# noamteyssier/sgcount

Hardware: NVIDIA B200
Metric: reads/sec matched per B200 (kernel & end-to-end) (higher is better)
Workload: dtype u8

## Files before the change

### sgcount_b200/csrc/common.cuh

```cuda
#pragma once

#include <cuda_runtime.h>
#include <stdint.h>

namespace sgc {

constexpr uint32_t kMaxK = 30;
constexpr uint32_t kNarrowMaxK = 20;
constexpr int kSeeds = 3;
constexpr int32_t kMiss = -1;

constexpr uint64_t kDirKindInline = 1ull << 62, kDirKindRun = 2ull << 62;
constexpr int kDirKindShift = 62;
constexpr uint32_t kDirStartMask = 0x3FFFFFu;

constexpr int kPostIdxShift = 40;

constexpr uint64_t kFrontFlag = 1ull << 40;
constexpr uint64_t kFrontOccupied = 1ull << 41;
constexpr int kFrontIdxShift = 42;

struct Key {
  uint32_t lo, hi;
};

__host__ __device__ __forceinline__ Key base_field(uint32_t j, bool wide) {
  const uint32_t word = j >> 2, byte = j & 3u;
  if (word < 4) return Key{3u << (8 * byte + 2 * word), 0u};
  return wide ? Key{0u, 3u << (8 * byte + 2 * (word - 4))} : Key{0u, 3u << (2 * byte)};
}
__host__ __device__ __forceinline__ void key_set_base(Key& k, uint32_t j, bool wide, uint32_t code) {
  const Key f = base_field(j, wide);
  k.lo = (k.lo & ~f.lo) | ((f.lo & (~f.lo + 1)) * code);
  k.hi = (k.hi & ~f.hi) | ((f.hi & (~f.hi + 1)) * code);
}
__host__ __device__ __forceinline__ uint32_t key_get_base(Key k, uint32_t j, bool wide) {
  const Key f = base_field(j, wide);
  return f.lo ? (k.lo & f.lo) / (f.lo & (~f.lo + 1)) : (k.hi & f.hi) / (f.hi & (~f.hi + 1));
}

constexpr uint32_t kFixedPartsMinK = 17;
struct SeedParts {
  uint32_t end[2];
  uint32_t keep_lo[kSeeds], keep_hi[kSeeds];
};
inline SeedParts make_seed_parts(uint32_t k, bool wide) {
  SeedParts sp{};
  const bool fixed = k >= kFixedPartsMinK;
  const uint32_t p0 = fixed ? 8 : (k + 2) / 3, p1 = fixed ? 8 : (k - p0 + 1) / 2;
  sp.end[0] = p0;
  sp.end[1] = p0 + p1;
  for (uint32_t j = 0; j < k; ++j) {
    const int part = j < sp.end[0] ? 0 : (j < sp.end[1] ? 1 : 2);
    const Key f = base_field(j, wide);
    for (int i = 0; i < kSeeds; ++i)
      if (i != part) {
        sp.keep_lo[i] |= f.lo;
        sp.keep_hi[i] |= f.hi;
      }
  }
  return sp;
}
__host__ __device__ __forceinline__ Key seed_of(const SeedParts& sp, Key k, int i) {
  return Key{k.lo & sp.keep_lo[i], k.hi & sp.keep_hi[i]};
}
__host__ __device__ __forceinline__ int part_of_base(const SeedParts& sp, uint32_t j) {
  return j < sp.end[0] ? 0 : (j < sp.end[1] ? 1 : 2);
}

template <bool FIXED>
__host__ __device__ __forceinline__ Key seed_of_t(const SeedParts& sp, Key k, int i) {
  if (FIXED) return i == 0 ? Key{k.lo & 0xF0F0F0F0u, k.hi} : (i == 1 ? Key{k.lo & 0x0F0F0F0Fu, k.hi} : Key{k.lo, 0u});
  return seed_of(sp, k, i);
}
template <bool FIXED>
__host__ __device__ __forceinline__ int part_of_base_t(const SeedParts& sp, uint32_t j) {
  if (FIXED) return j < 8 ? 0 : (j < 16 ? 1 : 2);
  return part_of_base(sp, j);
}
template <bool FIXED>
__host__ __device__ __forceinline__ uint32_t kept_difference(const SeedParts& sp, Key x, int list) {
  if (FIXED) {
    const uint32_t keep_lo = list == 0 ? 0xF0F0F0F0u : (list == 1 ? 0x0F0F0F0Fu : 0xFFFFFFFFu);
    return (x.lo & keep_lo) | (list < 2 ? x.hi : 0u);
  }
  return (x.lo & sp.keep_lo[list]) | (x.hi & sp.keep_hi[list]);
}

__host__ __device__ __forceinline__ uint32_t seed_hash(Key s) {
  uint32_t h = s.lo * 0x9E3779B1u + s.hi * 0x85EBCA77u;
  h ^= h >> 15;
  return h * 0x2C1B3C6Du;
}
__host__ __device__ __forceinline__ uint32_t front_hash(uint32_t lo, uint32_t hi) {
  return lo * 0x9E3779B1u + hi * 0x85EBCA77u;
}

__host__ __device__ __forceinline__ bool is_acgt(uint8_t c) {
  return c == 'A' || c == 'C' || c == 'G' || c == 'T';
}
__host__ __device__ __forceinline__ uint32_t code_of(uint8_t c) { return (c >> 1) & 3u; }

struct IndexView {
  const uint64_t* __restrict__ dir64[kSeeds];
  const ulonglong2* __restrict__ dir128[kSeeds];
  const uint64_t* __restrict__ post;
  const uint64_t* __restrict__ front;
};

struct LibView {
  uint32_t k, n;
  uint32_t wide;
  uint32_t dir_shift;
  uint32_t front_shift;
  SeedParts parts;
  IndexView fwd;
  IndexView rev;
};

#ifdef __CUDACC__

#ifndef SGC_L1_HINT
#define SGC_L1_HINT ""
#endif
__device__ __forceinline__ uint64_t ldg_u64(const uint64_t* p, uint64_t policy) {
  uint64_t v;
  asm volatile("ld.global.nc" SGC_L1_HINT ".L2::cache_hint.u64 %0, [%1], %2;" : "=l"(v) : "l"(p), "l"(policy));
  return v;
}
__device__ __forceinline__ uint32_t ldg_u32(const uint32_t* p, uint64_t policy) {
  uint32_t v;
  asm volatile("ld.global.nc" SGC_L1_HINT ".L2::cache_hint.u32 %0, [%1], %2;" : "=r"(v) : "l"(p), "l"(policy));
  return v;
}
__device__ __forceinline__ ulonglong2 ldg_u128(const ulonglong2* p, uint64_t policy) {
  ulonglong2 v;
  asm volatile("ld.global.nc" SGC_L1_HINT ".L2::cache_hint.v2.u64 {%0,%1}, [%2], %3;"
               : "=l"(v.x), "=l"(v.y)
               : "l"(p), "l"(policy));
  return v;
}
__device__ __forceinline__ void load_bucket(const uint64_t* p, uint64_t (&w)[4], uint64_t policy) {
  asm volatile("ld.global.nc" SGC_L1_HINT ".L2::cache_hint.v4.u64 {%0,%1,%2,%3}, [%4], %5;"
               : "=l"(w[0]), "=l"(w[1]), "=l"(w[2]), "=l"(w[3])
               : "l"(p), "l"(policy));
}
__device__ __forceinline__ uint64_t l2_evict_first_policy() {
  uint64_t pol;
  asm volatile("createpolicy.fractional.L2::evict_first.b64 %0, 1.0;" : "=l"(pol));
  return pol;
}
__device__ __forceinline__ uint64_t l2_evict_last_policy() {
  uint64_t pol;
  asm volatile("createpolicy.fractional.L2::evict_last.b64 %0, 1.0;" : "=l"(pol));
  return pol;
}

__device__ __forceinline__ int bases_differing(Key x) {
  return __popc((x.lo | (x.lo >> 1)) & 0x55555555u) + __popc((x.hi | (x.hi >> 1)) & 0x55555555u);
}

struct SeedRun {
  uint32_t first;
  uint32_t count;
};
__device__ __forceinline__ SeedRun seed_run128(const LibView& v, int seed, ulonglong2 entry) {
  SeedRun r;
  r.first = (uint32_t)seed * v.n + ((uint32_t)entry.y & kDirStartMask);
  r.count = (entry.x >> kDirKindShift) == 2 ? (uint32_t)(entry.y >> 22) : 0u;
  return r;
}
__device__ __forceinline__ SeedRun seed_run64(const LibView& v, int seed, uint64_t entry) {
  SeedRun r;
  r.first = (uint32_t)seed * v.n + ((uint32_t)entry & kDirStartMask);
  r.count = (entry >> kDirKindShift) == 2 ? (uint32_t)(entry >> 22) : 0u;
  return r;
}
template <bool WIDE>
__device__ __forceinline__ void load_posting(const IndexView& ix, uint32_t at, uint64_t policy, Key& key, uint32_t& idx) {
  if (WIDE) {
    const uint64_t w = ldg_u64(ix.post + 2 * (size_t)at, policy);
    key = Key{(uint32_t)w, (uint32_t)(w >> 32)};
    idx = (uint32_t)ldg_u64(ix.post + 2 * (size_t)at + 1, policy);
  } else {
    const uint64_t w = ldg_u64(ix.post + at, policy);
    key = Key{(uint32_t)w, (uint32_t)(w >> 32) & 0xFFu};
    idx = (uint32_t)(w >> kPostIdxShift) & 0x3FFFFFu;
  }
}

template <bool WIDE, typename F>
__device__ __forceinline__ void for_each_posting(const LibView& v, const IndexView& ix, int seed, Key key,
                                                 uint64_t policy, F&& visit) {
  const uint32_t h = seed_hash(seed_of(v.parts, key, seed));
  SeedRun r;
  if (WIDE) {
    const ulonglong2 e = ldg_u128(ix.dir128[seed] + (h >> v.dir_shift), policy);
    if ((e.x >> kDirKindShift) == 1) {
      visit(Key{(uint32_t)e.x, (uint32_t)(e.x >> 32) & 0x3FFFFFFFu}, (uint32_t)e.y);
      return;
    }
    r = seed_run128(v, seed, e);
  } else {
    const uint64_t e = ldg_u64(ix.dir64[seed] + (h >> v.dir_shift), policy);
    if ((e >> kDirKindShift) == 1) {
      visit(Key{(uint32_t)e, (uint32_t)(e >> 32) & 0xFFu}, (uint32_t)(e >> kPostIdxShift) & 0x3FFFFFu);
      return;
    }
    r = seed_run64(v, seed, e);
  }
#pragma unroll 1
  for (uint32_t c = 0; c < r.count; ++c) {
    Key mk;
    uint32_t idx;
    load_posting<WIDE>(ix, r.first + c, policy, mk, idx);
    if (visit(mk, idx)) break;
  }
}

template <bool WIDE, bool FIXED = false>
__device__ __forceinline__ int32_t lookup_token(const LibView& v, const IndexView& ix, bool with_perm, Key key, Key hole,
                                                int hole_list, bool active, int* kind, uint64_t policy) {
  static_assert(kSeeds == 3, "written for three lists");
  const bool wild = hole_list >= 0;
  int32_t found = kMiss;
  int parents = 0;
  bool member = false;
  auto consider = [&](int list, Key mk, uint32_t idx) {
    const Key x{(mk.lo ^ key.lo) & ~hole.lo, (mk.hi ^ key.hi) & ~hole.hi};
    if (kept_difference<FIXED>(v.parts, x, list) != 0) return;
    if ((x.lo | x.hi) == 0) {
      if (wild) {
        ++parents;
      } else {
        member = true;
      }
      found = (int32_t)idx;
    } else if (!wild && !member && bases_differing(x) == 1) {
      ++parents;
      found = (int32_t)idx;
    }
  };
  bool use[kSeeds];
  uint32_t h[kSeeds];
  SeedRun r[kSeeds];
#pragma unroll
  for (int i = 0; i < kSeeds; ++i) {
    use[i] = active && (wild ? i == hole_list : (i == 0 || with_perm));
    h[i] = seed_hash(seed_of_t<FIXED>(v.parts, key, i));
  }
  if (WIDE) {
    ulonglong2 entry[kSeeds];
#pragma unroll
    for (int i = 0; i < kSeeds; ++i)
      entry[i] = use[i] ? ldg_u128(ix.dir128[i] + (h[i] >> v.dir_shift), policy) : ulonglong2{0ull, 0ull};
#pragma unroll
    for (int i = 0; i < kSeeds; ++i) {
      if ((entry[i].x >> kDirKindShift) == 1)
        consider(i, Key{(uint32_t)entry[i].x, (uint32_t)(entry[i].x >> 32) & 0x3FFFFFFFu}, (uint32_t)entry[i].y);
      r[i] = seed_run128(v, i, entry[i]);
    }
  } else {
    uint64_t entry[kSeeds];
#pragma unroll
    for (int i = 0; i < kSeeds; ++i) entry[i] = use[i] ? ldg_u64(ix.dir64[i] + (h[i] >> v.dir_shift), policy) : 0ull;
#pragma unroll
    for (int i = 0; i < kSeeds; ++i) {
      if ((entry[i] >> kDirKindShift) == 1)
        consider(i, Key{(uint32_t)entry[i], (uint32_t)(entry[i] >> 32) & 0xFFu},
                 (uint32_t)(entry[i] >> kPostIdxShift) & 0x3FFFFFu);
      r[i] = seed_run64(v, i, entry[i]);
    }
  }
  const uint32_t end0 = r[0].count, end1 = end0 + r[1].count, total = end1 + r[2].count;
  const uint32_t base0 = r[0].first, base1 = r[1].first - end0, base2 = r[2].first - end1;
#pragma unroll 1
  for (uint32_t j = 0; j < total && !member; ++j) {
    const bool in0 = j < end0, in1 = j < end1;
    const uint32_t at = (in0 ? base0 : (in1 ? base1 : base2)) + j;
    Key mk;
    uint32_t idx;
    load_posting<WIDE>(ix, at, policy, mk, idx);
    consider(in0 ? 0 : (in1 ? 1 : 2), mk, idx);
  }
  if (member) {
    if (kind) *kind = 1;
    return found;
  }
  if (with_perm && parents == 1) {
    if (kind) *kind = 2;
    return found;
  }
  return kMiss;
}

template <bool WIDE>
__device__ __forceinline__ int32_t lookup_clean(const LibView& v, const IndexView& ix, bool with_perm, Key key,
                                                int* kind, uint64_t policy) {
  return lookup_token<WIDE>(v, ix, with_perm, key, Key{0u, 0u}, -1, true, kind, policy);
}

template <bool WIDE>
__device__ __forceinline__ int32_t lookup_wild(const LibView& v, const IndexView& ix, Key key, uint32_t pos, int* kind,
                                               uint64_t policy) {
  const Key hole = base_field(pos, WIDE);
  key.lo &= ~hole.lo;
  key.hi &= ~hole.hi;
  return lookup_token<WIDE>(v, ix, true, key, hole, part_of_base(v.parts, pos), true, kind, policy);
}

template <bool WIDE>
__device__ __forceinline__ int32_t window_lookup_t(const LibView& v, const IndexView& ix, bool with_perm, Key key,
                                                   int nbad, uint32_t bad_pos, bool bad_is_wild, int* kind,
                                                   uint64_t policy) {
  if (nbad == 0) return lookup_clean<WIDE>(v, ix, with_perm, key, kind, policy);
  if (nbad == 1 && bad_is_wild && with_perm) return lookup_wild<WIDE>(v, ix, key, bad_pos, kind, policy);
  return kMiss;
}

#endif

}
```

### sgcount_b200/csrc/count.cu

```cuda
#include <algorithm>
#include <cstdlib>
#include <mutex>
#include <set>
#include <utility>
#include <vector>

#include "internal.h"

namespace sgc {
namespace {

struct StreamGeom {
  int k, n, o;
  uint32_t with_perm;
  int win_src;
  int lead;
  uint32_t shift_bits[3];
  uint32_t try_plus, try_minus;
  int n_words;
  uint32_t last_mask;
  uint32_t wild_byte;
};

inline StreamGeom make_geom(uint32_t k, uint32_t read_len, int offset, bool with_perm, bool reverse, bool recursion,
                            int rc_mode) {
  StreamGeom g;
  g.k = (int)k;
  g.n = (int)read_len;
  g.o = offset;
  g.with_perm = with_perm;
  g.try_plus = recursion && g.o + 1 + g.k <= g.n;
  g.try_minus = g.try_plus && g.o >= 1;
  g.win_src = reverse ? g.n - g.o - g.k : g.o;
  const int d_plus = reverse ? -1 : 1;
  const bool before = (g.try_plus && d_plus < 0) || (g.try_minus && d_plus > 0);
  g.lead = before ? 1 : 0;
  g.shift_bits[0] = 8u * (uint32_t)g.lead;
  g.shift_bits[1] = 8u * (uint32_t)(g.lead + d_plus);
  g.shift_bits[2] = 8u * (uint32_t)(g.lead - d_plus);
  g.n_words = (g.k + 3) >> 2;
  g.last_mask = (g.k & 3) ? ((1u << (8 * (g.k & 3))) - 1) : ~0u;
  g.wild_byte = (reverse && rc_mode == SGC_RC_BITTRICK) ? (uint32_t)'J' : (uint32_t)'N';
  return g;
}

constexpr int kHotGuides = 4;

struct CountParams {
  LibView lib;
  const uint8_t* lines;
  const uint8_t* lines_end;
  const uint32_t* line_off;
  const uint32_t* line_end;
  uint64_t n_reads;
  uint64_t first_read;
  uint32_t stride, read_len;
  int offset;
  uint8_t with_perm, reverse, recursion, rc_mode;
  unsigned long long* state;
  unsigned long long* rep;
  uint32_t n_rep;
  uint32_t n_guides;
  int32_t hot[kHotGuides];
  uint32_t off_base;
  int32_t* assign_out;
  uint32_t debug;
  uint32_t zero;
  StreamGeom geom;
};

struct HotCounts {
  uint32_t c[kHotGuides];
};

template <int MODE>
__device__ __forceinline__ void flush_matched(const CountParams& p, uint32_t matched, const HotCounts& hot) {
  matched = __reduce_add_sync(0xffffffffu, matched);
  if ((threadIdx.x & 31) == 0 && matched) atomicAdd(p.state + p.n_guides + 1, (unsigned long long)matched);
  if (MODE == 4) {
#pragma unroll
    for (int j = 0; j < kHotGuides; ++j) {
      const uint32_t h = __reduce_add_sync(0xffffffffu, hot.c[j]);
      if ((threadIdx.x & 31) == 0 && h) atomicAdd(p.state + p.hot[j], (unsigned long long)h);
    }
  }
  if (blockIdx.x == 0 && threadIdx.x == 0) atomicAdd(p.state + p.n_guides, (unsigned long long)p.n_reads);
}

template <int MODE>
__device__ __forceinline__ void count_hit(const CountParams& p, unsigned long long* my_counts, int32_t hit,
                                          uint32_t& matched, HotCounts& hot) {
  if (hit >= 0) {
    ++matched;
    if (MODE == 4) {
      bool is_hot = false;
#pragma unroll
      for (int j = 0; j < kHotGuides; ++j) {
        const bool h = hit == p.hot[j];
        hot.c[j] += h;
        is_hot |= h;
      }
      if (!is_hot) atomicAdd(my_counts + hit, 1ull);
    } else {
      if (MODE != 2 || !(p.debug & 1u)) atomicAdd((MODE == 3 ? my_counts : p.state) + hit, 1ull);
    }
  }
}

__global__ void fold_replicas_kernel(unsigned long long* __restrict__ state, unsigned long long* __restrict__ rep,
                                     uint32_t n, uint32_t n_rep) {
  const uint32_t i = blockIdx.x * blockDim.x + threadIdx.x;
  if (i >= n) return;
  unsigned long long sum = 0;
  for (uint32_t r = 0; r < n_rep; ++r) {
    const unsigned long long v = rep[(size_t)r * n + i];
    if (v) {
      sum += v;
      rep[(size_t)r * n + i] = 0;
    }
  }
  if (sum) state[i] += sum;
}

constexpr int kWarpReads = 32;
constexpr int kMaxStages = 4;
#ifndef SGC_HANDBACK_MBAR
#define SGC_HANDBACK_MBAR 0
#endif
constexpr int kQueueCap = 64;
constexpr uint32_t kReadIdxBits = 30;

__device__ __forceinline__ uint32_t smem_u32(const void* p) { return (uint32_t)__cvta_generic_to_shared(p); }

__device__ __forceinline__ void mbar_init(uint64_t* bar, uint32_t count) {
  asm volatile("mbarrier.init.shared::cta.b64 [%0], %1;" ::"r"(smem_u32(bar)), "r"(count));
}
__device__ __forceinline__ void mbar_expect_tx(uint32_t bar, uint32_t bytes) {
  asm volatile("mbarrier.arrive.expect_tx.shared::cta.b64 _, [%0], %1;" ::"r"(bar), "r"(bytes) : "memory");
}
__device__ __forceinline__ void mbar_arrive(uint32_t bar) {
  asm volatile("mbarrier.arrive.shared::cta.b64 _, [%0];" ::"r"(bar) : "memory");
}
__device__ __forceinline__ void mbar_wait(uint32_t bar, uint32_t parity) {
  asm volatile(
      "{\n"
      ".reg .pred p;\n"
      "WAIT_LOOP:\n"
      "mbarrier.try_wait.parity.shared::cta.b64 p, [%0], %1;\n"
      "@p bra WAIT_DONE;\n"
      "bra WAIT_LOOP;\n"
      "WAIT_DONE:\n"
      "}\n" ::"r"(bar),
      "r"(parity)
      : "memory");
}
__device__ __forceinline__ void bulk_load(uint32_t dst, const void* src, uint32_t bytes, uint32_t bar, uint64_t policy) {
  asm volatile(
      "cp.async.bulk.shared::cluster.global.mbarrier::complete_tx::bytes.L2::cache_hint [%0], [%1], %2, [%3], %4;" ::
          "r"(dst),
      "l"(src), "r"(bytes), "r"(bar), "l"(policy)
      : "memory");
}
__device__ __forceinline__ bool elect_one() {
  uint32_t pred;
  asm volatile("{\n.reg .pred p;\nelect.sync _|p, 0xffffffff;\nselp.u32 %0, 1, 0, p;\n}\n" : "=r"(pred));
  return pred != 0;
}
template <int OFFSET>
__device__ __forceinline__ uint32_t lds_u32(uint32_t addr) {
  uint32_t v;
  asm volatile("ld.shared.u32 %0, [%1+%2];" : "=r"(v) : "r"(addr), "n"(OFFSET) : "memory");
  return v;
}
template <int I, int N>
struct LoadWords {
  static __device__ __forceinline__ void run(uint32_t addr, uint32_t* W) {
    W[I] = lds_u32<4 * I>(addr);
    LoadWords<I + 1, N>::run(addr, W);
  }
};
template <int N>
struct LoadWords<N, N> {
  static __device__ __forceinline__ void run(uint32_t, uint32_t*) {}
};

__device__ __forceinline__ uint32_t nonzero_byte_flags(uint32_t x) {
  return (((x & 0x7F7F7F7Fu) + 0x7F7F7F7Fu) | x) & 0x80808080u;
}

__device__ __forceinline__ uint32_t ascii_residue(uint32_t w) {
  const uint32_t is_t = (w >> 2) & ~(w >> 1) & 0x01010101u;
  return ((w & 0xF9F9F9F9u) ^ (is_t * 0x11u)) ^ 0x41414141u;
}

template <int NW, bool WIDE>
__device__ __forceinline__ uint32_t pack_window(const uint32_t (&w)[NW], int n_words, uint32_t last_mask, Key& key,
                                                uint32_t (&x)[NW]) {
  uint32_t lo = 0, hi = 0, any = 0;
#pragma unroll
  for (int i = 0; i < NW; ++i) {
    x[i] = ascii_residue(w[i]);
    uint32_t c = (w[i] >> 1) & 0x03030303u;
    if (NW >= 5) {
      if (i == NW - 1) {
        x[i] &= last_mask;
        c &= last_mask;
      }
    } else {
      const uint32_t mk = i < n_words - 1 ? ~0u : (i == n_words - 1 ? last_mask : 0u);
      x[i] &= mk;
      c &= mk;
    }
    any |= x[i];
    if (i < 4)
      lo += c << (2 * i);
    else
      hi += c << (2 * (i - 4));
  }
  if (!WIDE) hi = (hi * 0x01041040u) >> 24;
  key = Key{lo, hi};
  return any;
}

template <int NW>
struct WarpQueueT {
  uint32_t w[NW + 1][kQueueCap];
  uint32_t tag[kQueueCap];
};

template <int NW, bool WIDE>
__device__ __forceinline__ int32_t try_position(const LibView& v, const IndexView& ix, const StreamGeom& g,
                                                const uint32_t (&S)[NW + 1], uint32_t shift, uint64_t policy,
                                                uint32_t debug = 0) {
  uint32_t w[NW], x[NW];
#pragma unroll
  for (int i = 0; i < NW; ++i) w[i] = __funnelshift_r(S[i], S[i + 1], shift);
  Key key;
  const uint32_t any = pack_window<NW, WIDE>(w, g.n_words, g.last_mask, key, x);
  if (debug & 8u) return (key.lo == 0x12345678u && any == 77u) ? 0 : kMiss;
  int nbad = 0;
  uint32_t bad_word = 0, bad_flags = 0, bad_w = 0;
#pragma unroll
  for (int i = 0; i < NW; ++i) {
    const uint32_t f = nonzero_byte_flags(x[i]);
    nbad += __popc(f);
    if (f) {
      bad_word = (uint32_t)i;
      bad_flags = f;
      bad_w = w[i];
    }
  }
  const uint32_t byte = ((uint32_t)(__ffs((int)bad_flags) - 8) >> 3) & 3u;
  const bool wild = g.with_perm && nbad == 1 && ((bad_w >> (8 * byte)) & 0xFFu) == g.wild_byte;
  const uint32_t pos = wild ? 4 * bad_word + byte : 0u;
  Key hole{0u, 0u};
  if (wild) {
    hole = base_field(pos, WIDE);
    key.lo &= ~hole.lo;
    key.hi &= ~hole.hi;
  }
  constexpr bool kFixedParts = NW == 5 || WIDE;
  static_assert(kFixedPartsMinK <= 17, "k = 17..30 must use the fixed parts");
  return lookup_token<WIDE, kFixedParts>(v, ix, g.with_perm, key, hole,
                                         wild ? part_of_base_t<kFixedParts>(v.parts, pos) : -1, any == 0 || wild,
                                         nullptr, policy);
}

__device__ __forceinline__ uint64_t ldg_stream_u64(const uint64_t* p, uint64_t policy) {
  uint64_t v;
  asm volatile("ld.global.nc.L2::cache_hint.u64 %0, [%1], %2;" : "=l"(v) : "l"(p), "l"(policy));
  return v;
}

constexpr uint32_t kLineIdxBits = 27;
constexpr uint32_t kLineLead = 1u << 27, kLinePlus = 1u << 28, kLineMinus = 1u << 29;
constexpr int kLineWarps = 8;

template <int NW, bool WIDE>
__global__ void __launch_bounds__(kLineWarps * 32) count_lines_kernel(CountParams p) {
  __shared__ WarpQueueT<NW> queues[kLineWarps];
  const int lane = threadIdx.x & 31, warp = threadIdx.x >> 5;
  WarpQueueT<NW>* q = &queues[warp];
  uint32_t matched = 0;
  HotCounts hot{};
  const uint64_t table_policy = l2_evict_last_policy();
  const uint64_t line_policy = l2_evict_first_policy();
  const int k = (int)p.lib.k;
  const StreamGeom& g = p.geom;
  const IndexView& ix = p.reverse ? p.lib.rev : p.lib.fwd;
  const uint32_t gwarp = blockIdx.x * kLineWarps + warp, gwarps = gridDim.x * kLineWarps;
  unsigned long long* my_counts = p.rep + (size_t)(gwarp & (p.n_rep - 1)) * p.n_guides;
  const int d_plus = p.reverse ? -1 : 1;
  constexpr int NL = (4 * NW + 11 + 7) / 8;
  static_assert(2 * NL >= NW + 3, "span words");
  uint32_t qn = 0;

  auto settle = [&](int32_t hit, uint32_t ridx) {
    if (p.assign_out) p.assign_out[p.first_read + ridx] = hit;
    count_hit<4>(p, my_counts, hit, matched, hot);
  };
  auto drain = [&](bool all) {
    while (qn >= 32 || (all && qn > 0)) {
      const uint32_t cnt = qn < 32 ? qn : 32;
      qn -= cnt;
      int next = -1;
      uint32_t S[NW + 1], tag = 0;
      if ((uint32_t)lane < cnt) {
        const uint32_t e = qn + lane;
#pragma unroll
        for (int i = 0; i < NW + 1; ++i) S[i] = q->w[i][e];
        tag = q->tag[e];
        const uint32_t pos = tag >> 30, ridx = tag & ((1u << kLineIdxBits) - 1);
        const int lead = (tag & kLineLead) ? 1 : 0;
        const uint32_t shift = 8u * (uint32_t)(pos == 0 ? lead : (pos == 1 ? lead + d_plus : lead - d_plus));
        const int32_t hit = try_position<NW, WIDE>(p.lib, ix, g, S, shift, table_policy);
        if (hit == kMiss) next = pos == 0 ? ((tag & kLinePlus) ? 1 : -1) : (pos == 1 && (tag & kLineMinus) ? 2 : -1);
        if (next < 0) settle(hit, ridx);
      }
      __syncwarp();
      const uint32_t pm = __ballot_sync(0xffffffffu, next >= 0);
      if (pm) {
        if (next >= 0) {
          const uint32_t e = qn + __popc(pm & ((1u << lane) - 1));
#pragma unroll
          for (int i = 0; i < NW + 1; ++i) q->w[i][e] = S[i];
          q->tag[e] = ((uint32_t)next << 30) | (tag & 0x3FFFFFFFu);
        }
        qn += __popc(pm);
      }
      __syncwarp();
    }
  };

  const uint64_t n_tiles = (p.n_reads + 31) / 32;
  for (uint64_t t = gwarp; t < n_tiles; t += gwarps) {
    const uint64_t i = t * 32 + lane;
    int park = -1;
    uint32_t S[NW + 1] = {}, flags = 0;
    if (i < p.n_reads) {
      const uint64_t r = p.first_read + i;
      uint64_t start;
      int n;
      if (p.line_end) {
        start = p.line_off[r];
        n = (int)(p.line_end[r] - p.line_off[r]);
      } else if (p.line_off) {
        const uint32_t a = p.line_off[r], b = p.line_off[r + 1];
        start = a - p.off_base;
        n = (int)(b - a) - 1;
      } else {
        start = r * p.stride;
        n = (int)p.read_len;
      }
      if (p.offset + k > n) {
        settle(kMiss, (uint32_t)i);
      } else {
        const bool try_plus = p.recursion && p.offset + 1 + k <= n;
        const bool try_minus = try_plus && p.offset >= 1;
        const int win_src = p.reverse ? n - p.offset - k : p.offset;
        const int lead = ((try_plus && d_plus < 0) || (try_minus && d_plus > 0)) ? 1 : 0;
        flags = (lead ? kLineLead : 0u) | (try_plus ? kLinePlus : 0u) | (try_minus ? kLineMinus : 0u);
        const uint8_t* sb = p.lines + start + win_src - lead;
        const uint64_t* a8 = reinterpret_cast<const uint64_t*>((uintptr_t)sb & ~(uintptr_t)7);
        uint32_t R[2 * NL];
#pragma unroll
        for (int j = 0; j < NL; ++j) {
          const uint64_t v =
              reinterpret_cast<const uint8_t*>(a8 + j) < p.lines_end ? ldg_stream_u64(a8 + j, line_policy) : 0ull;
          R[2 * j] = (uint32_t)v;
          R[2 * j + 1] = (uint32_t)(v >> 32);
        }
        const uint32_t sh = (uint32_t)((uintptr_t)sb & 7u);
        const bool odd = (sh & 4u) != 0;
        const uint32_t bits = (sh & 3u) * 8u;
#pragma unroll
        for (int j = 0; j < NW + 1; ++j) {
          const uint32_t w0 = odd ? R[j + 1] : R[j], w1 = odd ? R[j + 2] : R[j + 1];
          S[j] = __funnelshift_r(w0, w1, bits);
        }
        uint32_t w[NW], x[NW];
#pragma unroll
        for (int j = 0; j < NW; ++j) w[j] = __funnelshift_r(S[j], S[j + 1], 8u * (uint32_t)lead);
        Key key;
        const uint32_t any = pack_window<NW, WIDE>(w, g.n_words, g.last_mask, key, x);
        park = 0;
        if (any == 0) {
          uint64_t b[4];
          load_bucket(ix.front + (size_t)(front_hash(key.lo, key.hi) >> p.lib.front_shift) * 4, b, table_policy);
          bool found, flagged;
          int32_t idx;
          if (!WIDE) {
            uint32_t sel = 0;
#pragma unroll
            for (int j = 3; j >= 0; --j)
              if ((uint32_t)b[j] == key.lo) sel = (uint32_t)(b[j] >> 32);
            const uint32_t want = key.hi | (uint32_t)(kFrontOccupied >> 32);
            found = ((sel ^ want) & (0xFFu | (uint32_t)(kFrontOccupied >> 32))) == 0;
            idx = (int32_t)(sel >> (kFrontIdxShift - 32));
            flagged = (b[0] & kFrontFlag) != 0;
          } else {
            const uint64_t probe = ((uint64_t)key.hi << 32) | key.lo;
            const bool m0 = b[0] == probe && (b[1] & kFrontOccupied), m1 = b[2] == probe && (b[3] & kFrontOccupied);
            found = m0 || m1;
            idx = (int32_t)((m0 ? b[1] : b[3]) >> kFrontIdxShift);
            flagged = (b[1] & kFrontFlag) != 0;
          }
          if (found) {
            park = -1;
            settle(idx, (uint32_t)i);
          } else if (!flagged && !g.with_perm) {
            park = try_plus ? 1 : -1;
            if (park < 0) settle(kMiss, (uint32_t)i);
          }
        } else if (!g.with_perm) {
          park = try_plus ? 1 : -1;
          if (park < 0) settle(kMiss, (uint32_t)i);
        }
      }
    }
    const uint32_t pm = __ballot_sync(0xffffffffu, park >= 0);
    if (pm) {
      if (park >= 0) {
        const uint32_t e = qn + __popc(pm & ((1u << lane) - 1));
#pragma unroll
        for (int j = 0; j < NW + 1; ++j) q->w[j][e] = S[j];
        q->tag[e] = ((uint32_t)park << 30) | flags | (uint32_t)i;
      }
      qn += __popc(pm);
      __syncwarp();
    }
    drain(false);
  }
  drain(true);
  flush_matched<4>(p, matched, hot);
}

template <int NW, bool WIDE, int MODE>
__global__ void __launch_bounds__(384, 2) count_stream_kernel(const CountParams p, uint32_t n_wtiles, int n_stages,
                                                              uint32_t stage_bytes) {
  extern __shared__ __align__(128) uint8_t smem[];
  const int lane = threadIdx.x & 31;
  const int warp = __shfl_sync(0xffffffffu, (int)(threadIdx.x >> 5), 0);
  const int warps_per_cta = blockDim.x >> 5;
  uint8_t* my_tiles = smem + (size_t)warp * n_stages * stage_bytes;
  uint64_t* bars = reinterpret_cast<uint64_t*>(smem + (size_t)warps_per_cta * n_stages * stage_bytes);
  uint64_t* my_bar = bars + warp * (2 * kMaxStages);
  WarpQueueT<NW>* q = reinterpret_cast<WarpQueueT<NW>*>(bars + warps_per_cta * (2 * kMaxStages)) + warp;

  const uint32_t tile_bytes = kWarpReads * p.stride;
  const uint32_t gwarp = blockIdx.x * warps_per_cta + warp;
  const uint32_t gwarps = gridDim.x * warps_per_cta;
  const uint64_t src_step = (uint64_t)gwarps * tile_bytes;
  const uint8_t* next_src = p.lines + (uint64_t)gwarp * tile_bytes;

  const uint32_t tiles_sm = smem_u32(my_tiles), bars_sm = smem_u32(my_bar);
  const uint64_t policy = l2_evict_first_policy();
  uint32_t requested = gwarp;
  if (lane == 0) {
    for (int s = 0; s < n_stages; ++s) {
      mbar_init(&my_bar[s], 1);
      mbar_init(&my_bar[kMaxStages + s], 32);
    }
    asm volatile("fence.mbarrier_init.release.cluster;" ::: "memory");
    asm volatile("fence.proxy.async.shared::cta;" ::: "memory");
  }
  __syncwarp();
  for (int s = 0; s < n_stages; ++s) {
    if (requested < n_wtiles) {
      if (elect_one()) {
        mbar_expect_tx(bars_sm + 8u * (uint32_t)s, tile_bytes);
        bulk_load(tiles_sm + (uint32_t)s * stage_bytes, next_src, tile_bytes, bars_sm + 8u * (uint32_t)s, policy);
      }
      requested += gwarps;
      next_src += src_step;
    }
  }

  const StreamGeom& g = p.geom;
  const uint32_t sbyte = (uint32_t)lane * p.stride + (uint32_t)(g.win_src - g.lead);
  const uint32_t lane_off = sbyte & ~3u;
  const uint32_t off_bits = (sbyte & 3u) * 8;
  const uint32_t win_bits = off_bits + g.shift_bits[0];
  const IndexView& ix = p.reverse ? p.lib.rev : p.lib.fwd;
  const uint64_t* __restrict__ front = ix.front;
  const uint32_t front_shift = p.lib.front_shift;
  const uint64_t table_policy = l2_evict_last_policy();
  const uint32_t debug = MODE == 2 ? p.debug : 0u;
  const bool centered_again = g.with_perm;
  const bool any_next = centered_again || g.try_plus;

  uint32_t matched = 0;
  HotCounts hot{};
  unsigned long long* my_counts = p.rep + (size_t)(gwarp & (p.n_rep - 1)) * p.n_guides;
  uint32_t qn = 0;
  int s = 0;
  uint32_t parity = 0;
  uint32_t cur_tile = tiles_sm, cur_bar = bars_sm;

  struct Pending {
    uint32_t S[NW + 1];
    Key key;
    uint32_t any;
  };
  uint64_t bucket[4];
  auto fetch_bucket = [&](const Pending& pd) {
    if (pd.any == 0 && !(MODE == 2 && (debug & 2u)))
      load_bucket(front + (size_t)(front_hash(pd.key.lo, pd.key.hi) >> front_shift) * 4, bucket, table_policy);
  };
  auto settle = [&](int32_t hit, uint32_t ridx) {
    if ((MODE == 1 || MODE == 2) && p.assign_out) p.assign_out[ridx] = hit;
    count_hit<MODE>(p, my_counts, hit, matched, hot);
  };
  auto step_a = [&](Pending& pd) {
    mbar_wait(cur_bar, parity);
    uint32_t W[NW + 2];
    LoadWords<0, NW + 2>::run(cur_tile + lane_off, W);
#if SGC_HANDBACK_MBAR
    if (requested < n_wtiles) {
      mbar_arrive(cur_bar + 8u * kMaxStages);
      if (elect_one()) {
        mbar_wait(cur_bar + 8u * kMaxStages, parity);
        mbar_expect_tx(cur_bar, tile_bytes);
        bulk_load(cur_tile, next_src, tile_bytes, cur_bar, policy);
      }
      requested += gwarps;
      next_src += src_step;
    }
#else
    uint32_t allw = W[0];
#pragma unroll
    for (int i = 1; i < NW + 2; ++i) allw &= W[i];
    const uint32_t arrived = __ballot_sync(0xffffffffu, allw != 0) & p.zero;
    if (requested < n_wtiles) {
      if (elect_one()) {
        mbar_expect_tx(cur_bar, tile_bytes + arrived);
        bulk_load(cur_tile, next_src, tile_bytes + arrived, cur_bar, policy);
      }
      requested += gwarps;
      next_src += src_step;
    }
#endif
    cur_tile += stage_bytes;
    cur_bar += 8;
    if (++s == n_stages) {
      s = 0;
      parity ^= 1u;
      cur_tile = tiles_sm;
      cur_bar = bars_sm;
    }
#pragma unroll
    for (int i = 0; i < NW + 1; ++i) pd.S[i] = __funnelshift_r(W[i], W[i + 1], off_bits);
    uint32_t w[NW], x[NW];
#pragma unroll
    for (int i = 0; i < NW; ++i) w[i] = __funnelshift_r(pd.S[i], pd.S[i + 1], g.shift_bits[0]);
    pd.any = pack_window<NW, WIDE>(w, g.n_words, g.last_mask, pd.key, x);
  };
  auto step_b = [&](const Pending& pd, uint32_t read_idx) {
    int park = 0;
    if (pd.any == 0) {
      bool found, flagged;
      int32_t hit;
      if (MODE == 2 && (debug & 2u)) {
        found = true;
// ... 679 lines not shown
```

Baseline: 62.54 billion.

## Unroll posting walk by two and make lookup bookkeeping branchless

The posting-list walk now fetches two postings per iteration before evaluating them, so their global loads can be in flight together. The per-candidate consider logic becomes predicated, with no early returns. In try_position the wildcard hole mask is built branchlessly from per-word flags instead of calling base_field. The cost is extra work on short runs, where predicated-off slots are still evaluated, plus some added register pressure.

```diff
diff --git a/sgcount_b200/csrc/common.cuh b/sgcount_b200/csrc/common.cuh
--- a/sgcount_b200/csrc/common.cuh
+++ b/sgcount_b200/csrc/common.cuh
@@ -189,6 +189,11 @@
   }
 }
 
+#ifndef SGC_WALK_STEP
+#define SGC_WALK_STEP 2
+#endif
+constexpr uint32_t kWalkStep = SGC_WALK_STEP;
+
 template <bool WIDE, typename F>
 __device__ __forceinline__ void for_each_posting(const LibView& v, const IndexView& ix, int seed, Key key,
                                                  uint64_t policy, F&& visit) {
@@ -226,20 +231,15 @@
   int32_t found = kMiss;
   int parents = 0;
   bool member = false;
-  auto consider = [&](int list, Key mk, uint32_t idx) {
+  auto consider = [&](int list, bool valid, Key mk, uint32_t idx) {
     const Key x{(mk.lo ^ key.lo) & ~hole.lo, (mk.hi ^ key.hi) & ~hole.hi};
-    if (kept_difference<FIXED>(v.parts, x, list) != 0) return;
-    if ((x.lo | x.hi) == 0) {
-      if (wild) {
-        ++parents;
-      } else {
-        member = true;
-      }
-      found = (int32_t)idx;
-    } else if (!wild && !member && bases_differing(x) == 1) {
-      ++parents;
-      found = (int32_t)idx;
-    }
+    const bool kept = valid && kept_difference<FIXED>(v.parts, x, list) == 0;
+    const bool same = (x.lo | x.hi) == 0;
+    const bool is_member = kept && same && !wild;
+    const bool is_parent = kept && (wild ? same : !member && bases_differing(x) == 1);
+    parents += is_parent;
+    member |= is_member;
+    found = is_member || is_parent ? (int32_t)idx : found;
   };
   bool use[kSeeds];
   uint32_t h[kSeeds];
@@ -256,8 +256,8 @@
       entry[i] = use[i] ? ldg_u128(ix.dir128[i] + (h[i] >> v.dir_shift), policy) : ulonglong2{0ull, 0ull};
 #pragma unroll
     for (int i = 0; i < kSeeds; ++i) {
-      if ((entry[i].x >> kDirKindShift) == 1)
-        consider(i, Key{(uint32_t)entry[i].x, (uint32_t)(entry[i].x >> 32) & 0x3FFFFFFFu}, (uint32_t)entry[i].y);
+      consider(i, (entry[i].x >> kDirKindShift) == 1,
+               Key{(uint32_t)entry[i].x, (uint32_t)(entry[i].x >> 32) & 0x3FFFFFFFu}, (uint32_t)entry[i].y);
       r[i] = seed_run128(v, i, entry[i]);
     }
   } else {
@@ -266,22 +266,30 @@
     for (int i = 0; i < kSeeds; ++i) entry[i] = use[i] ? ldg_u64(ix.dir64[i] + (h[i] >> v.dir_shift), policy) : 0ull;
 #pragma unroll
     for (int i = 0; i < kSeeds; ++i) {
-      if ((entry[i] >> kDirKindShift) == 1)
-        consider(i, Key{(uint32_t)entry[i], (uint32_t)(entry[i] >> 32) & 0xFFu},
-                 (uint32_t)(entry[i] >> kPostIdxShift) & 0x3FFFFFu);
+      consider(i, (entry[i] >> kDirKindShift) == 1, Key{(uint32_t)entry[i], (uint32_t)(entry[i] >> 32) & 0xFFu},
+               (uint32_t)(entry[i] >> kPostIdxShift) & 0x3FFFFFu);
       r[i] = seed_run64(v, i, entry[i]);
     }
   }
   const uint32_t end0 = r[0].count, end1 = end0 + r[1].count, total = end1 + r[2].count;
   const uint32_t base0 = r[0].first, base1 = r[1].first - end0, base2 = r[2].first - end1;
 #pragma unroll 1
-  for (uint32_t j = 0; j < total && !member; ++j) {
-    const bool in0 = j < end0, in1 = j < end1;
-    const uint32_t at = (in0 ? base0 : (in1 ? base1 : base2)) + j;
-    Key mk;
-    uint32_t idx;
-    load_posting<WIDE>(ix, at, policy, mk, idx);
-    consider(in0 ? 0 : (in1 ? 1 : 2), mk, idx);
+  for (uint32_t j = 0; j < total && !member; j += kWalkStep) {
+    Key mk[kWalkStep];
+    uint32_t idx[kWalkStep];
+#pragma unroll
+    for (uint32_t u = 0; u < kWalkStep; ++u) {
+      const uint32_t c = j + u;
+      const uint32_t at = (c < end0 ? base0 : (c < end1 ? base1 : base2)) + c;
+      mk[u] = Key{0u, 0u};
+      idx[u] = 0;
+      if (c < total) load_posting<WIDE>(ix, at, policy, mk[u], idx[u]);
+    }
+#pragma unroll
+    for (uint32_t u = 0; u < kWalkStep; ++u) {
+      const uint32_t c = j + u;
+      consider(c < end0 ? 0 : (c < end1 ? 1 : 2), c < total, mk[u], idx[u]);
+    }
   }
   if (member) {
     if (kind) *kind = 1;
diff --git a/sgcount_b200/csrc/count.cu b/sgcount_b200/csrc/count.cu
--- a/sgcount_b200/csrc/count.cu
+++ b/sgcount_b200/csrc/count.cu
@@ -240,25 +240,28 @@
   if (debug & 8u) return (key.lo == 0x12345678u && any == 77u) ? 0 : kMiss;
   int nbad = 0;
   uint32_t bad_word = 0, bad_flags = 0, bad_w = 0;
+  Key field{0u, 0u};
 #pragma unroll
   for (int i = 0; i < NW; ++i) {
     const uint32_t f = nonzero_byte_flags(x[i]);
     nbad += __popc(f);
-    if (f) {
-      bad_word = (uint32_t)i;
-      bad_flags = f;
-      bad_w = w[i];
-    }
+    bad_word = f ? (uint32_t)i : bad_word;
+    bad_flags = f ? f : bad_flags;
+    bad_w = f ? w[i] : bad_w;
+    const uint32_t lsb = (f >> 7) * 3u;
+    if (i < 4)
+      field.lo |= lsb << (2 * i);
+    else if (WIDE)
+      field.hi |= lsb << (2 * (i - 4));
+    else
+      field.hi |= (lsb * 0x01041040u) >> 24;
   }
   const uint32_t byte = ((uint32_t)(__ffs((int)bad_flags) - 8) >> 3) & 3u;
   const bool wild = g.with_perm && nbad == 1 && ((bad_w >> (8 * byte)) & 0xFFu) == g.wild_byte;
-  const uint32_t pos = wild ? 4 * bad_word + byte : 0u;
-  Key hole{0u, 0u};
-  if (wild) {
-    hole = base_field(pos, WIDE);
-    key.lo &= ~hole.lo;
-    key.hi &= ~hole.hi;
-  }
+  const uint32_t pos = 4 * bad_word + byte;
+  const Key hole{wild ? field.lo : 0u, wild ? field.hi : 0u};
+  key.lo &= ~hole.lo;
+  key.hi &= ~hole.hi;
   constexpr bool kFixedParts = NW == 5 || WIDE;
   static_assert(kFixedPartsMinK <= 17, "k = 17..30 must use the fixed parts");
   return lookup_token<WIDE, kFixedParts>(v, ix, g.with_perm, key, hole,
```

Result: no change. 62.73 billion (median of 6 runs) (+0.3%).
